# raulmur/ORB_SLAM2

Hardware: NVIDIA H100
Metric: stereo frames/sec (ORB extract L+R + ComputeStereoMatches, KITTI-shaped 1242x375 @2000 kpts) (higher is better)
Workload: dtype u8

## Files before the change

orb_slam2_b200/csrc/k_fast.cu:

```cuda
#include <cuda.h>

#include <cstring>

#include "borb_internal.h"

#include <algorithm>
#include <vector>

namespace borb {

namespace {

constexpr int TP = 160;
constexpr int TROWS = 66;
constexpr int QCAP = 60 * 128;

__device__ __forceinline__ uint32_t smem_u32(const void* p) { return (uint32_t)__cvta_generic_to_shared(p); }

template <int DX>
__device__ __forceinline__ uint32_t win(uint32_t W0, uint32_t W1, uint32_t W2) {
    if (DX == 0) return W1;
    if (DX > 0) return __byte_perm(W1, W2, DX | ((DX + 1) << 4) | ((DX + 2) << 8) | ((DX + 3) << 12));
    constexpr int K = 4 + DX;
    return __byte_perm(W0, W1, K | ((K + 1) << 4) | ((K + 2) << 8) | ((K + 3) << 12));
}

__device__ __forceinline__ uint32_t gt_flag(uint32_t q, uint32_t v, uint32_t K) {
    const uint32_t a = __vabsdiffu4(q, v);
    return (a + K) | a;
}

__device__ __forceinline__ uint32_t score_word(const uint32_t (&R0)[7], const uint32_t (&R1)[7], const uint32_t (&R2)[7]) {
#define ROWJ(dy) R0[(dy) + 3], R1[(dy) + 3], R2[(dy) + 3]
    uint32_t wn[16];
    wn[0] = win<0>(ROWJ(3));    wn[1] = win<1>(ROWJ(3));    wn[2] = win<2>(ROWJ(2));     wn[3] = win<3>(ROWJ(1));
    wn[4] = win<3>(ROWJ(0));    wn[5] = win<3>(ROWJ(-1));   wn[6] = win<2>(ROWJ(-2));    wn[7] = win<1>(ROWJ(-3));
    wn[8] = win<0>(ROWJ(-3));   wn[9] = win<-1>(ROWJ(-3));  wn[10] = win<-2>(ROWJ(-2));  wn[11] = win<-3>(ROWJ(-1));
    wn[12] = win<-3>(ROWJ(0));  wn[13] = win<-3>(ROWJ(1));  wn[14] = win<-2>(ROWJ(2));   wn[15] = win<-1>(ROWJ(3));
#undef ROWJ
    const uint32_t v = R1[3];
    uint32_t res[2];
#pragma unroll
    for (int half = 0; half < 2; half++) {
        const uint32_t v2 = half ? __byte_perm(v, 0u, 0x4341) : (v & 0x00FF00FFu);
        const uint32_t nv2 = __vneg2(v2);
        uint32_t d[16];
#pragma unroll
        for (int k = 0; k < 16; k++) {
            const uint32_t q2 = half ? __byte_perm(wn[k], 0u, 0x4341) : (wn[k] & 0x00FF00FFu);
            d[k] = __vadd2(q2, nv2);
        }
        uint32_t lo3[16], hi3[16];
#pragma unroll
        for (int k = 0; k < 16; k++) {
            lo3[k] = __vimin3_s16x2(d[k], d[(k + 1) & 15], d[(k + 2) & 15]);
            hi3[k] = __vimax3_s16x2(d[k], d[(k + 1) & 15], d[(k + 2) & 15]);
        }
        uint32_t lo9[16], hi9[16];
#pragma unroll
        for (int k = 0; k < 16; k++) {
            lo9[k] = __vimin3_s16x2(lo3[k], lo3[(k + 3) & 15], lo3[(k + 6) & 15]);
            hi9[k] = __vimax3_s16x2(hi3[k], hi3[(k + 3) & 15], hi3[(k + 6) & 15]);
        }
        uint32_t bb[5], dd[5];
#pragma unroll
        for (int k = 0; k < 5; k++) {
            bb[k] = __vimax3_s16x2(lo9[3 * k], lo9[3 * k + 1], lo9[3 * k + 2]);
            dd[k] = __vimin3_s16x2(hi9[3 * k], hi9[3 * k + 1], hi9[3 * k + 2]);
        }
        const uint32_t bright = __vimax3_s16x2(__vimax3_s16x2(bb[0], bb[1], bb[2]), __vimax3_s16x2(bb[3], bb[4], lo9[15]), bb[0]);
        const uint32_t darkm = __vimin3_s16x2(__vimin3_s16x2(dd[0], dd[1], dd[2]), __vimin3_s16x2(dd[3], dd[4], hi9[15]), dd[0]);
        res[half] = __viaddmax_s16x2_relu(__vmaxs2(bright, __vneg2(darkm)), 0xFFFFFFFFu, 0u);
    }
    return res[1] * 256u + res[0];
}

}

struct TMaps { CUtensorMap m[BORB_MAX_LEVELS]; };

struct __align__(16) FastTile { int16_t l, ncell, x0, x1, y0, y1, wCell, hCell; };

__global__ void __launch_bounds__(256, 4) fast_kernel(const __grid_constant__ Geometry g, const __grid_constant__ TMaps tm,
                                                   const FastTile* __restrict__ tiles, uint32_t* __restrict__ cand, int* __restrict__ cand_cnt) {
    __shared__ __align__(128) uint8_t tile[TROWS * TP];
    __shared__ __align__(16) uint8_t score[60 * TP];
    __shared__ uint16_t queue[QCAP];
    __shared__ uint16_t wqueue[8 * 256];
    __shared__ int wcnt[8];
    __shared__ __align__(8) unsigned long long bar;
    __shared__ uint32_t scoredRow[60];
    __shared__ int qn, needB;
    __shared__ int cellHasIni[128 / 30 + 1];
    __shared__ uint8_t cellOf[128];

    const int img = blockIdx.y;
    const FastTile T = tiles[blockIdx.x];
    const int l = T.l, ncell = T.ncell, x0 = T.x0, x1 = T.x1, y0 = T.y0, y1 = T.y1;
    const int wCell = T.wCell, hCell = T.hCell;
    const LevelGeom& L = g.lv[l];
    const int tw = x1 - x0, th = y1 - y0;
    const int tid = threadIdx.x;
    const int lane = tid & 31, wrp = tid >> 5;

    const int xs = (x0 - 4) & ~15;
    const int off = x0 - xs;
    if (tid == 0) {
        asm volatile("mbarrier.init.shared::cta.b64 [%0], 1;" ::"r"(smem_u32(&bar)));
        asm volatile("fence.mbarrier_init.release.cluster;" ::: "memory");
        const uint32_t bytes = (uint32_t)TP * (uint32_t)(hCell + 6);
        asm volatile("mbarrier.arrive.expect_tx.shared::cta.b64 _, [%0], %1;" ::"r"(smem_u32(&bar)), "r"(bytes) : "memory");
        asm volatile(
            "cp.async.bulk.tensor.3d.shared::cluster.global.tile.mbarrier::complete_tx::bytes [%0], [%1, {%2, %3, %4}], [%5];"
            ::"r"(smem_u32(tile)), "l"(reinterpret_cast<uint64_t>(&tm.m[l])), "r"(xs), "r"(y0 - 3), "r"(img), "r"(smem_u32(&bar))
            : "memory");
    }
    if (tid < 128 / 30 + 1) cellHasIni[tid] = 0;
    if (tid < 128) cellOf[tid] = (uint8_t)(tid / wCell);
    if (tid == 0) { qn = 0; needB = 0; }
    __syncthreads();
    asm volatile(
        "{\n"
        ".reg .pred p;\n"
        "FAST_TMA_WAIT:\n"
        "mbarrier.try_wait.parity.shared::cta.b64 p, [%0], 0;\n"
        "@p bra FAST_TMA_DONE;\n"
        "bra FAST_TMA_WAIT;\n"
        "FAST_TMA_DONE:\n"
        "}\n" ::"r"(smem_u32(&bar))
        : "memory");
    if (g.fast_mode == 1) {
        if (reinterpret_cast<const uint32_t*>(tile)[tid] == 0x12345678u && cand_cnt[0] == -1) cand[0] = 1;
        return;
    }

    const int tlow = g.ini_th;
    const uint32_t* T32 = reinterpret_cast<const uint32_t*>(tile);
    uint32_t* S32 = reinterpret_cast<uint32_t*>(score);
    const int wbase = off >> 2;
    const uint32_t T1 = (uint32_t)(127 - min(tlow, 127)) * 0x01010101u;
    const uint32_t TC = (uint32_t)min(max(tlow, 1), 128) * 0x01010101u;
    const bool reject_ok = tlow <= 127;

    auto commit = [&](uint32_t sw, int yy, int wc, bool write, int tlow, uint32_t TC, uint32_t needMask) {
        const int col = 4 * wc;
        uint32_t vm = 0;
#pragma unroll
        for (int b = 0; b < 4; b++)
            if (col + b - off >= 0 && col + b - off < tw) vm |= 0x80u << (8 * b);
        if (write) S32[yy * (TP / 4) + wc] = sw;
        uint32_t m = (((sw | 0x80808080u) - TC) | sw) & vm & needMask;
        if (tlow > 128) {
            m = 0;
#pragma unroll
            for (int b = 0; b < 4; b++)
                if ((int)((sw >> (8 * b)) & 0xFF) >= tlow) m |= 0x80u << (8 * b);
            m &= vm & needMask;
        }
        if (!write) m = 0;
        const unsigned any = __ballot_sync(0xFFFFFFFFu, m != 0);
        if (any) {
            const int c = __popc(m);
            int incl = c;
#pragma unroll
            for (int o2 = 1; o2 < 32; o2 <<= 1) {
                const int t = __shfl_up_sync(0xFFFFFFFFu, incl, o2);
                if (lane >= o2) incl += t;
            }
            int base = 0;
            if (lane == 31) base = atomicAdd(&qn, incl);
            base = __shfl_sync(0xFFFFFFFFu, base, 31) + incl - c;
            uint32_t mm = m;
            while (mm) {
                const int b = (__ffs(mm) - 1) >> 3;
                mm &= mm - 1;
                queue[base++] = (uint16_t)((yy << 8) | (col + b));
            }
        }
    };

    {
        const int RG = (th + 7) >> 3;
        const int yBeg = wrp * RG, yEnd = min(th, yBeg + RG);
        const int wc = wbase + lane;
        uint32_t vmask = 0;
#pragma unroll
        for (int b = 0; b < 4; b++)
            if (4 * wc + b - off >= 0 && 4 * wc + b - off < tw) vmask |= 0x80u << (8 * b);
        uint32_t a0[7], a1[7], a2[7];
        int wcount = 0;
        if (yBeg < yEnd) {
#pragma unroll
            for (int j = 0; j < 6; j++) {
                const uint32_t* rp = T32 + (yBeg + j) * (TP / 4) + wc - 1;
                a0[j] = rp[0]; a1[j] = rp[1]; a2[j] = rp[2];
            }
        }
#pragma unroll
        for (int it = 0; it < 8; it++) {
            const int yy = yBeg + it;
            if (yy < yEnd) {
                {
                    const uint32_t* rp = T32 + (yy + 6) * (TP / 4) + wc - 1;
                    a0[(it + 6) % 7] = rp[0]; a1[(it + 6) % 7] = rp[1]; a2[(it + 6) % 7] = rp[2];
                }
#define ROW(dy) a0[(it + (dy) + 3) % 7], a1[(it + (dy) + 3) % 7], a2[(it + (dy) + 3) % 7]
                bool keep = vmask != 0;
                if (reject_ok && keep) {
                    const uint32_t v = a1[(it + 3) % 7];
                    uint32_t acc = gt_flag(win<0>(ROW(3)), v, T1) | gt_flag(win<0>(ROW(-3)), v, T1);
                    acc &= gt_flag(win<2>(ROW(2)), v, T1) | gt_flag(win<-2>(ROW(-2)), v, T1);
                    acc &= gt_flag(win<3>(ROW(0)), v, T1) | gt_flag(win<-3>(ROW(0)), v, T1);
                    acc &= gt_flag(win<2>(ROW(-2)), v, T1) | gt_flag(win<-2>(ROW(2)), v, T1);
                    keep = (acc & vmask) != 0;
                }
#undef ROW
                const unsigned bal = __ballot_sync(0xFFFFFFFFu, keep);
                if (lane == 0) scoredRow[yy] = bal;
                if (!keep && vmask != 0) S32[yy * (TP / 4) + wc] = 0;
                if (keep) wqueue[wrp * 256 + wcount + __popc(bal & ((1u << lane) - 1))] = (uint16_t)((yy << 5) | lane);
                wcount += __popc(bal);
            }
        }
        if (lane == 0) wcnt[wrp] = wcount;
    }
    __syncthreads();
    if (g.fast_mode == 2) {
        if (wcnt[0] == -1) cand[0] = 1;
        return;
    }

    {
        int c[8], nw = 0;
#pragma unroll
        for (int w = 0; w < 8; w++) { c[w] = wcnt[w]; nw += c[w]; }
        for (int eb = 0; eb < nw; eb += 256) {
            const int e = eb + tid;
            uint32_t sw = 0;
            int yy = 0, wc = wbase;
            const bool have = e < nw;
            if (have) {
                int seg = 0, r = e;
#pragma unroll
                for (int w = 0; w < 7; w++)
                    if (seg == w && r >= c[w]) { r -= c[w]; seg = w + 1; }
                const int we = wqueue[seg * 256 + r];
                yy = we >> 5;
                wc = wbase + (we & 31);
                uint32_t R0[7], R1[7], R2[7];
#pragma unroll
                for (int j = 0; j < 7; j++) {
                    const uint32_t* rp = T32 + (yy + j) * (TP / 4) + wc - 1;
                    R0[j] = rp[0]; R1[j] = rp[1]; R2[j] = rp[2];
                }
                sw = score_word(R0, R1, R2);
            }
            commit(sw, yy, wc, have, tlow, TC, 0xFFFFFFFFu);
        }
    }
    __syncthreads();
    int nq = qn;
    if (g.fast_mode == 3) {
        if (nq == -1) cand[0] = 1;
        return;
    }

    uint32_t* out = cand + (size_t)img * g.cand_image_stride + L.cand_off;
    int* cnt = cand_cnt + img * g.nlevels + l;

    auto nms = [&](int n, bool mark) {
        for (int e = tid; e < n; e += 256) {
            const int q = queue[e];
            const int col = q & 255, yy = q >> 8;
            const int xx = col - off;
            const int s = score[yy * TP + col];
            const int c = cellOf[xx];
            const int cx0 = c * wCell, cx1 = min(cx0 + wCell, tw);
            bool ismax = true;
#pragma unroll
            for (int dy = -1; dy <= 1; dy++)
#pragma unroll
                for (int dx = -1; dx <= 1; dx++) {
                    if (dx == 0 && dy == 0) continue;
                    const int qx = xx + dx, qy = yy + dy;
                    if (qx < cx0 || qx >= cx1 || qy < 0 || qy >= th) continue;
                    if (!(s > (int)score[qy * TP + col + dx])) ismax = false;
                }
            if (ismax) {
                if (mark) cellHasIni[c] = 1;
            } else
                queue[e] = 0xFFFF;
        }
    };
    auto emit = [&](int n) {
        for (int eb = 0; eb < n; eb += 256) {
            const int e = eb + tid;
            int s = 0, xx = 0, yy = 0;
            if (e < n) {
                const int q = queue[e];
                if (q != 0xFFFF) {
                    const int col = q & 255;
                    yy = q >> 8; xx = col - off;
                    s = score[yy * TP + col];
                }
            }
            const unsigned m = __ballot_sync(0xFFFFFFFFu, s > 0);
            if (m) {
                int base = 0;
                if (lane == 0) base = atomicAdd(cnt, __popc(m));
                base = __shfl_sync(0xFFFFFFFFu, base, 0);
                if (s > 0) {
                    const int pos = base + __popc(m & ((1u << lane) - 1));
                    if (pos < L.cand_cap) out[pos] = pack_xys(x0 + xx, y0 + yy, s);
                }
            }
        }
    };

    nms(nq, true);
    __syncthreads();
    emit(nq);
    if (tid < ncell && tid * wCell < tw && !cellHasIni[tid] && g.min_th < g.ini_th) needB = 1;
    __syncthreads();
    if (!needB) return;

    {
        if (tid == 0) qn = 0;
        __syncthreads();
        const int tmin = g.min_th;
        const uint32_t T1b = (uint32_t)(127 - min(tmin, 127)) * 0x01010101u;
        const uint32_t TCb = (uint32_t)min(max(tmin, 1), 128) * 0x01010101u;
        const int nwords = th * 32;
        for (int wb = 0; wb < nwords; wb += 256) {
            const int widx = wb + tid;
            const int yy = widx >> 5;
            const int wc = wbase + (widx & 31);
            uint32_t needMask = 0, sw = 0;
            bool write = false;
            if (widx < nwords) {
#pragma unroll
                for (int b = 0; b < 4; b++) {
                    const int xx = 4 * wc + b - off;
                    if (xx >= 0 && xx < tw && !cellHasIni[cellOf[xx]]) needMask |= 0x80u << (8 * b);
                }
                if (needMask) {
                    write = true;
                    if ((scoredRow[yy] >> (widx & 31)) & 1u) {
                        sw = S32[yy * (TP / 4) + wc];
                    } else {
                        uint32_t R0[7], R1[7], R2[7];
#pragma unroll
                        for (int j = 0; j < 7; j++) {
                            const uint32_t* rp = T32 + (yy + j) * (TP / 4) + wc - 1;
                            R0[j] = rp[0]; R1[j] = rp[1]; R2[j] = rp[2];
                        }
                        bool keep = true;
                        if (tmin <= 127) {
                            const uint32_t v = R1[3];
#define ROWJ(dy) R0[(dy) + 3], R1[(dy) + 3], R2[(dy) + 3]
                            uint32_t acc = gt_flag(win<0>(ROWJ(3)), v, T1b) | gt_flag(win<0>(ROWJ(-3)), v, T1b);
                            acc &= gt_flag(win<2>(ROWJ(2)), v, T1b) | gt_flag(win<-2>(ROWJ(-2)), v, T1b);
                            acc &= gt_flag(win<3>(ROWJ(0)), v, T1b) | gt_flag(win<-3>(ROWJ(0)), v, T1b);
                            acc &= gt_flag(win<2>(ROWJ(-2)), v, T1b) | gt_flag(win<-2>(ROWJ(2)), v, T1b);
#undef ROWJ
                            keep = (acc & 0x80808080u) != 0;
                        }
                        sw = keep ? score_word(R0, R1, R2) : 0u;
                    }
                }
            }
            commit(sw, yy, wc, write, tmin, TCb, needMask);
        }
        __syncthreads();
        nq = qn;
        nms(nq, false);
        __syncthreads();
        emit(nq);
    }
}

typedef CUresult (*EncodeTiledFn)(CUtensorMap*, CUtensorMapDataType, cuuint32_t, void*, const cuuint64_t*, const cuuint64_t*,
                                  const cuuint32_t*, const cuuint32_t*, CUtensorMapInterleave, CUtensorMapSwizzle,
                                  CUtensorMapL2promotion, CUtensorMapFloatOOBfill);

borb_status build_fast_tmaps(const Geometry& g, const Workspace& ws, void* out_tmaps) {
    static EncodeTiledFn encode = nullptr;
    if (!encode) {
        void* fn = nullptr;
        cudaDriverEntryPointQueryResult qres;
        cudaError_t e = cudaGetDriverEntryPoint("cuTensorMapEncodeTiled", &fn, cudaEnableDefault, &qres);
        if (e != cudaSuccess || qres != cudaDriverEntryPointSuccess || !fn) {
            set_error("cuTensorMapEncodeTiled unavailable (%s)", cudaGetErrorString(e));
            return BORB_ERR_CUDA;
        }
        encode = (EncodeTiledFn)fn;
    }
    TMaps* tm = reinterpret_cast<TMaps*>(out_tmaps);
    std::memset(tm, 0, sizeof(TMaps));
    for (int l = 0; l < g.nlevels; l++) {
        const LevelGeom& L = g.lv[l];
        cuuint64_t dims[3] = {(cuuint64_t)L.w, (cuuint64_t)L.h, (cuuint64_t)ws.max_images};
        cuuint64_t strides[2] = {(cuuint64_t)L.pitch, (cuuint64_t)g.pyr_image_stride};
        cuuint32_t box[3] = {(cuuint32_t)TP, (cuuint32_t)(L.hCell + 6), 1};
        cuuint32_t estr[3] = {1, 1, 1};
        CUresult r = encode(&tm->m[l], CU_TENSOR_MAP_DATA_TYPE_UINT8, 3, ws.pyr + L.pyr_off, dims, strides, box, estr,
                            CU_TENSOR_MAP_INTERLEAVE_NONE, CU_TENSOR_MAP_SWIZZLE_NONE, CU_TENSOR_MAP_L2_PROMOTION_L2_128B,
                            CU_TENSOR_MAP_FLOAT_OOB_FILL_NONE);
        if (r != CUDA_SUCCESS) {
            set_error("cuTensorMapEncodeTiled failed for level %d (CUresult %d)", l, (int)r);
            return BORB_ERR_CUDA;
        }
    }
    return BORB_OK;
}

size_t fast_tmaps_bytes() { return sizeof(TMaps); }

borb_status build_fast_tiles(const Geometry& g, Workspace& ws) {
    std::vector<FastTile> t;
    for (int l = 0; l < g.nlevels; l++) {
        const LevelGeom& L = g.lv[l];
        for (int cellRow = 0; cellRow < L.nRows; cellRow++)
            for (int blkCol = 0; blkCol < L.blkCols; blkCol++) {
                const int cell0 = blkCol * L.cellsPerBlk;
                const int ncell = std::min(L.cellsPerBlk, L.nCols - cell0);
                const int x0 = EDGE + cell0 * L.wCell, x1 = std::min(x0 + ncell * L.wCell, L.w - EDGE);
                const int y0 = EDGE + cellRow * L.hCell, y1 = std::min(y0 + L.hCell, L.h - EDGE);
                if (x0 >= x1 || y0 >= y1) continue;
                FastTile f;
                f.l = (int16_t)l; f.ncell = (int16_t)ncell; f.x0 = (int16_t)x0; f.x1 = (int16_t)x1; f.y0 = (int16_t)y0; f.y1 = (int16_t)y1;
                f.wCell = (int16_t)L.wCell; f.hCell = (int16_t)L.hCell;
                t.push_back(f);
            }
    }
    cudaFree(ws.fast_tiles); ws.fast_tiles = nullptr;
    ws.fast_n_tiles = (int)t.size();
    if (t.empty()) return BORB_OK;
    BORB_CUDA(cudaMalloc(&ws.fast_tiles, t.size() * sizeof(FastTile)));
    BORB_CUDA(cudaMemcpy(ws.fast_tiles, t.data(), t.size() * sizeof(FastTile), cudaMemcpyHostToDevice));
    return BORB_OK;
}

int launch_fast(const Geometry& g, const Workspace& ws, int n_images, cudaStream_t s) {
    if (ws.fast_n_tiles == 0) return 0;
    dim3 grid(ws.fast_n_tiles, n_images);
    fast_kernel<<<grid, 256, 0, s>>>(g, *reinterpret_cast<const TMaps*>(ws.fast_tmaps), reinterpret_cast<const FastTile*>(ws.fast_tiles), ws.cand, ws.cand_cnt);
    return 1;
}

}
```

Before: 35610.

## Score FAST corners per surviving pixel instead of per 4-pixel word

FAST scoring is restructured. The old path scored whole 4-byte words whenever any pixel in the word passed the rejection test. The new path records per-pixel survivor flags in a warp queue, compacts the individual pixels into a block-wide queue, and scores two pixels per thread with a scalar 16-bit pair routine reading bytes from shared memory. The low-threshold pass reuses the same collect/score path and drops the scoredRow cache, so previously scored words are recomputed. This cuts wasted scoring on non-candidate pixels but adds an extra compaction stage, byte-granular shared loads and extra block syncs inside the scoring loop.

```diff
diff --git a/orb_slam2_b200/csrc/k_fast.cu b/orb_slam2_b200/csrc/k_fast.cu
--- a/orb_slam2_b200/csrc/k_fast.cu
+++ b/orb_slam2_b200/csrc/k_fast.cu
@@ -30,49 +30,40 @@
     return (a + K) | a;
 }
 
-__device__ __forceinline__ uint32_t score_word(const uint32_t (&R0)[7], const uint32_t (&R1)[7], const uint32_t (&R2)[7]) {
-#define ROWJ(dy) R0[(dy) + 3], R1[(dy) + 3], R2[(dy) + 3]
-    uint32_t wn[16];
-    wn[0] = win<0>(ROWJ(3));    wn[1] = win<1>(ROWJ(3));    wn[2] = win<2>(ROWJ(2));     wn[3] = win<3>(ROWJ(1));
-    wn[4] = win<3>(ROWJ(0));    wn[5] = win<3>(ROWJ(-1));   wn[6] = win<2>(ROWJ(-2));    wn[7] = win<1>(ROWJ(-3));
-    wn[8] = win<0>(ROWJ(-3));   wn[9] = win<-1>(ROWJ(-3));  wn[10] = win<-2>(ROWJ(-2));  wn[11] = win<-3>(ROWJ(-1));
-    wn[12] = win<-3>(ROWJ(0));  wn[13] = win<-3>(ROWJ(1));  wn[14] = win<-2>(ROWJ(2));   wn[15] = win<-1>(ROWJ(3));
-#undef ROWJ
-    const uint32_t v = R1[3];
-    uint32_t res[2];
-#pragma unroll
-    for (int half = 0; half < 2; half++) {
-        const uint32_t v2 = half ? __byte_perm(v, 0u, 0x4341) : (v & 0x00FF00FFu);
-        const uint32_t nv2 = __vneg2(v2);
-        uint32_t d[16];
-#pragma unroll
-        for (int k = 0; k < 16; k++) {
-            const uint32_t q2 = half ? __byte_perm(wn[k], 0u, 0x4341) : (wn[k] & 0x00FF00FFu);
-            d[k] = __vadd2(q2, nv2);
-        }
-        uint32_t lo3[16], hi3[16];
-#pragma unroll
-        for (int k = 0; k < 16; k++) {
-            lo3[k] = __vimin3_s16x2(d[k], d[(k + 1) & 15], d[(k + 2) & 15]);
-            hi3[k] = __vimax3_s16x2(d[k], d[(k + 1) & 15], d[(k + 2) & 15]);
-        }
-        uint32_t lo9[16], hi9[16];
-#pragma unroll
-        for (int k = 0; k < 16; k++) {
-            lo9[k] = __vimin3_s16x2(lo3[k], lo3[(k + 3) & 15], lo3[(k + 6) & 15]);
-            hi9[k] = __vimax3_s16x2(hi3[k], hi3[(k + 3) & 15], hi3[(k + 6) & 15]);
-        }
-        uint32_t bb[5], dd[5];
-#pragma unroll
-        for (int k = 0; k < 5; k++) {
-            bb[k] = __vimax3_s16x2(lo9[3 * k], lo9[3 * k + 1], lo9[3 * k + 2]);
-            dd[k] = __vimin3_s16x2(hi9[3 * k], hi9[3 * k + 1], hi9[3 * k + 2]);
-        }
-        const uint32_t bright = __vimax3_s16x2(__vimax3_s16x2(bb[0], bb[1], bb[2]), __vimax3_s16x2(bb[3], bb[4], lo9[15]), bb[0]);
-        const uint32_t darkm = __vimin3_s16x2(__vimin3_s16x2(dd[0], dd[1], dd[2]), __vimin3_s16x2(dd[3], dd[4], hi9[15]), dd[0]);
-        res[half] = __viaddmax_s16x2_relu(__vmaxs2(bright, __vneg2(darkm)), 0xFFFFFFFFu, 0u);
-    }
-    return res[1] * 256u + res[0];
+__device__ __forceinline__ uint32_t score_pair(const uint32_t (&d)[16], uint32_t v2) {
+    uint32_t lo3[16], hi3[16];
+#pragma unroll
+    for (int k = 0; k < 16; k++) {
+        lo3[k] = __vimin3_s16x2(d[k], d[(k + 1) & 15], d[(k + 2) & 15]);
+        hi3[k] = __vimax3_s16x2(d[k], d[(k + 1) & 15], d[(k + 2) & 15]);
+    }
+    uint32_t lo9[16], hi9[16];
+#pragma unroll
+    for (int k = 0; k < 16; k++) {
+        lo9[k] = __vimin3_s16x2(lo3[k], lo3[(k + 3) & 15], lo3[(k + 6) & 15]);
+        hi9[k] = __vimax3_s16x2(hi3[k], hi3[(k + 3) & 15], hi3[(k + 6) & 15]);
+    }
+    uint32_t bb[5], dd[5];
+#pragma unroll
+    for (int k = 0; k < 5; k++) {
+        bb[k] = __vimax3_s16x2(lo9[3 * k], lo9[3 * k + 1], lo9[3 * k + 2]);
+        dd[k] = __vimin3_s16x2(hi9[3 * k], hi9[3 * k + 1], hi9[3 * k + 2]);
+    }
+    const uint32_t bright = __vimax3_s16x2(__vimax3_s16x2(bb[0], bb[1], bb[2]), __vimax3_s16x2(bb[3], bb[4], lo9[15]), bb[0]);
+    const uint32_t darkm = __vimin3_s16x2(__vimin3_s16x2(dd[0], dd[1], dd[2]), __vimin3_s16x2(dd[3], dd[4], hi9[15]), dd[0]);
+    return __viaddmax_s16x2_relu(__vmaxs2(__vsub2(bright, v2), __vsub2(v2, darkm)), 0xFFFFFFFFu, 0u);
+}
+
+__device__ __forceinline__ uint32_t score_pixels(const uint8_t* pa, const uint8_t* pb) {
+    constexpr int RX[16] = {0, 1, 2, 3, 3, 3, 2, 1, 0, -1, -2, -3, -3, -3, -2, -1};
+    constexpr int RY[16] = {3, 3, 2, 1, 0, -1, -2, -3, -3, -3, -2, -1, 0, 1, 2, 3};
+    uint32_t d[16];
+#pragma unroll
+    for (int k = 0; k < 16; k++) {
+        const int o = RY[k] * TP + RX[k];
+        d[k] = (uint32_t)pa[o] | ((uint32_t)pb[o] << 16);
+    }
+    return score_pair(d, (uint32_t)pa[0] | ((uint32_t)pb[0] << 16));
 }
 
 }
@@ -86,11 +77,9 @@
     __shared__ __align__(128) uint8_t tile[TROWS * TP];
     __shared__ __align__(16) uint8_t score[60 * TP];
     __shared__ uint16_t queue[QCAP];
-    __shared__ uint16_t wqueue[8 * 256];
-    __shared__ int wcnt[8];
+    __shared__ uint32_t wqueue[8 * 256];
     __shared__ __align__(8) unsigned long long bar;
-    __shared__ uint32_t scoredRow[60];
-    __shared__ int qn, needB;
+    __shared__ int pn, qn, needB;
     __shared__ int cellHasIni[128 / 30 + 1];
     __shared__ uint8_t cellOf[128];
 
@@ -117,7 +106,7 @@
     }
     if (tid < 128 / 30 + 1) cellHasIni[tid] = 0;
     if (tid < 128) cellOf[tid] = (uint8_t)(tid / wCell);
-    if (tid == 0) { qn = 0; needB = 0; }
+    if (tid == 0) { pn = 0; qn = 0; needB = 0; }
     __syncthreads();
     asm volatile(
         "{\n"
@@ -134,59 +123,21 @@
         return;
     }
 
-    const int tlow = g.ini_th;
     const uint32_t* T32 = reinterpret_cast<const uint32_t*>(tile);
     uint32_t* S32 = reinterpret_cast<uint32_t*>(score);
     const int wbase = off >> 2;
-    const uint32_t T1 = (uint32_t)(127 - min(tlow, 127)) * 0x01010101u;
-    const uint32_t TC = (uint32_t)min(max(tlow, 1), 128) * 0x01010101u;
-    const bool reject_ok = tlow <= 127;
-
-    auto commit = [&](uint32_t sw, int yy, int wc, bool write, int tlow, uint32_t TC, uint32_t needMask) {
-        const int col = 4 * wc;
-        uint32_t vm = 0;
-#pragma unroll
-        for (int b = 0; b < 4; b++)
-            if (col + b - off >= 0 && col + b - off < tw) vm |= 0x80u << (8 * b);
-        if (write) S32[yy * (TP / 4) + wc] = sw;
-        uint32_t m = (((sw | 0x80808080u) - TC) | sw) & vm & needMask;
-        if (tlow > 128) {
-            m = 0;
-#pragma unroll
-            for (int b = 0; b < 4; b++)
-                if ((int)((sw >> (8 * b)) & 0xFF) >= tlow) m |= 0x80u << (8 * b);
-            m &= vm & needMask;
-        }
-        if (!write) m = 0;
-        const unsigned any = __ballot_sync(0xFFFFFFFFu, m != 0);
-        if (any) {
-            const int c = __popc(m);
-            int incl = c;
-#pragma unroll
-            for (int o2 = 1; o2 < 32; o2 <<= 1) {
-                const int t = __shfl_up_sync(0xFFFFFFFFu, incl, o2);
-                if (lane >= o2) incl += t;
-            }
-            int base = 0;
-            if (lane == 31) base = atomicAdd(&qn, incl);
-            base = __shfl_sync(0xFFFFFFFFu, base, 31) + incl - c;
-            uint32_t mm = m;
-            while (mm) {
-                const int b = (__ffs(mm) - 1) >> 3;
-                mm &= mm - 1;
-                queue[base++] = (uint16_t)((yy << 8) | (col + b));
-            }
-        }
-    };
-
-    {
+    const int wc = wbase + lane;
+    uint32_t vmask = 0;
+#pragma unroll
+    for (int b = 0; b < 4; b++)
+        if (4 * wc + b - off >= 0 && 4 * wc + b - off < tw) vmask |= 0x80u << (8 * b);
+
+    auto collect = [&](int t, uint32_t m, bool zero) {
+        const uint32_t K = (uint32_t)(127 - min(t, 127)) * 0x01010101u;
+        asm volatile("" : "+r"(m));
+        const bool reject = t <= 127;
         const int RG = (th + 7) >> 3;
         const int yBeg = wrp * RG, yEnd = min(th, yBeg + RG);
-        const int wc = wbase + lane;
-        uint32_t vmask = 0;
-#pragma unroll
-        for (int b = 0; b < 4; b++)
-            if (4 * wc + b - off >= 0 && 4 * wc + b - off < tw) vmask |= 0x80u << (8 * b);
         uint32_t a0[7], a1[7], a2[7];
         int wcount = 0;
         if (yBeg < yEnd) {
@@ -205,59 +156,84 @@
                     a0[(it + 6) % 7] = rp[0]; a1[(it + 6) % 7] = rp[1]; a2[(it + 6) % 7] = rp[2];
                 }
 #define ROW(dy) a0[(it + (dy) + 3) % 7], a1[(it + (dy) + 3) % 7], a2[(it + (dy) + 3) % 7]
-                bool keep = vmask != 0;
-                if (reject_ok && keep) {
+                uint32_t f = m;
+                if (reject && m) {
                     const uint32_t v = a1[(it + 3) % 7];
-                    uint32_t acc = gt_flag(win<0>(ROW(3)), v, T1) | gt_flag(win<0>(ROW(-3)), v, T1);
-                    acc &= gt_flag(win<2>(ROW(2)), v, T1) | gt_flag(win<-2>(ROW(-2)), v, T1);
-                    acc &= gt_flag(win<3>(ROW(0)), v, T1) | gt_flag(win<-3>(ROW(0)), v, T1);
-                    acc &= gt_flag(win<2>(ROW(-2)), v, T1) | gt_flag(win<-2>(ROW(2)), v, T1);
-                    keep = (acc & vmask) != 0;
+                    uint32_t acc = gt_flag(win<0>(ROW(3)), v, K) | gt_flag(win<0>(ROW(-3)), v, K);
+                    acc &= gt_flag(win<2>(ROW(2)), v, K) | gt_flag(win<-2>(ROW(-2)), v, K);
+                    acc &= gt_flag(win<3>(ROW(0)), v, K) | gt_flag(win<-3>(ROW(0)), v, K);
+                    acc &= gt_flag(win<2>(ROW(-2)), v, K) | gt_flag(win<-2>(ROW(2)), v, K);
+                    f = acc & m;
                 }
 #undef ROW
-                const unsigned bal = __ballot_sync(0xFFFFFFFFu, keep);
-                if (lane == 0) scoredRow[yy] = bal;
-                if (!keep && vmask != 0) S32[yy * (TP / 4) + wc] = 0;
-                if (keep) wqueue[wrp * 256 + wcount + __popc(bal & ((1u << lane) - 1))] = (uint16_t)((yy << 5) | lane);
+                const unsigned bal = __ballot_sync(0xFFFFFFFFu, f != 0);
+                if (zero && m != 0) S32[yy * (TP / 4) + wc] = 0;
+                if (f) wqueue[wrp * 256 + wcount + __popc(bal & ((1u << lane) - 1))] = f | (uint32_t)(yy << 8) | (uint32_t)wc;
                 wcount += __popc(bal);
             }
         }
-        if (lane == 0) wcnt[wrp] = wcount;
-    }
+        __syncwarp();
+        for (int i = 0; i < wcount; i += 32) {
+            const uint32_t we = i + lane < wcount ? wqueue[wrp * 256 + i + lane] : 0u;
+            const uint32_t fl = we & 0x80808080u;
+            const int c = __popc(fl);
+            int incl = c;
+#pragma unroll
+            for (int o2 = 1; o2 < 32; o2 <<= 1) {
+                const int s = __shfl_up_sync(0xFFFFFFFFu, incl, o2);
+                if (lane >= o2) incl += s;
+            }
+            int base = 0;
+            if (lane == 31) base = atomicAdd(&pn, incl);
+            base = __shfl_sync(0xFFFFFFFFu, base, 31) + incl - c;
+            const int e = (int)((we >> 8) & 63) << 8 | (int)(4 * (we & 127));
+#pragma unroll
+            for (int b = 0; b < 4; b++)
+                if (fl & (0x80u << (8 * b))) queue[base++] = (uint16_t)(e + b);
+        }
+    };
+
+    auto score_queue = [&](int t) {
+        const int np = pn;
+        const int tc = max(t, 1);
+        for (int rb = 0; rb < np; rb += 512) {
+            const int e0 = rb + wrp * 64 + lane, e1 = e0 + 32;
+            const bool va = e0 < np, vb = e1 < np;
+            const int qa = va ? queue[e0] : off;
+            const int qb = vb ? queue[e1] : qa;
+            __syncthreads();
+            if (rb + wrp * 64 < np) {
+                const int ia = (qa >> 8) * TP + (qa & 255), ib = (qb >> 8) * TP + (qb & 255);
+                const uint32_t s2 = score_pixels(tile + ia + 3 * TP, tile + ib + 3 * TP);
+                const int sa = (int)(s2 & 0xFFFFu), sb = (int)(s2 >> 16);
+                if (va) score[ia] = (uint8_t)sa;
+                if (vb) score[ib] = (uint8_t)sb;
+                const bool ca = va && sa >= tc, cb = vb && sb >= tc;
+                if (__any_sync(0xFFFFFFFFu, ca || cb)) {
+                    const int c = (int)ca + (int)cb;
+                    int incl = c;
+#pragma unroll
+                    for (int o2 = 1; o2 < 32; o2 <<= 1) {
+                        const int s = __shfl_up_sync(0xFFFFFFFFu, incl, o2);
+                        if (lane >= o2) incl += s;
+                    }
+                    int base = 0;
+                    if (lane == 31) base = atomicAdd(&qn, incl);
+                    base = __shfl_sync(0xFFFFFFFFu, base, 31) + incl - c;
+                    if (ca) queue[base++] = (uint16_t)qa;
+                    if (cb) queue[base] = (uint16_t)qb;
+                }
+            }
+        }
+    };
+
+    collect(g.ini_th, vmask, true);
     __syncthreads();
     if (g.fast_mode == 2) {
-        if (wcnt[0] == -1) cand[0] = 1;
+        if (pn == -1) cand[0] = 1;
         return;
     }
-
-    {
-        int c[8], nw = 0;
-#pragma unroll
-        for (int w = 0; w < 8; w++) { c[w] = wcnt[w]; nw += c[w]; }
-        for (int eb = 0; eb < nw; eb += 256) {
-            const int e = eb + tid;
-            uint32_t sw = 0;
-            int yy = 0, wc = wbase;
-            const bool have = e < nw;
-            if (have) {
-                int seg = 0, r = e;
-#pragma unroll
-                for (int w = 0; w < 7; w++)
-                    if (seg == w && r >= c[w]) { r -= c[w]; seg = w + 1; }
-                const int we = wqueue[seg * 256 + r];
-                yy = we >> 5;
-                wc = wbase + (we & 31);
-                uint32_t R0[7], R1[7], R2[7];
-#pragma unroll
-                for (int j = 0; j < 7; j++) {
-                    const uint32_t* rp = T32 + (yy + j) * (TP / 4) + wc - 1;
-                    R0[j] = rp[0]; R1[j] = rp[1]; R2[j] = rp[2];
-                }
-                sw = score_word(R0, R1, R2);
-            }
-            commit(sw, yy, wc, have, tlow, TC, 0xFFFFFFFFu);
-        }
-    }
+    score_queue(g.ini_th);
     __syncthreads();
     int nq = qn;
     if (g.fast_mode == 3) {
@@ -325,52 +301,17 @@
     if (!needB) return;
 
     {
-        if (tid == 0) qn = 0;
+        uint32_t need = 0;
+#pragma unroll
+        for (int b = 0; b < 4; b++) {
+            const int xx = 4 * wc + b - off;
+            if (xx >= 0 && xx < tw && !cellHasIni[cellOf[xx]]) need |= 0x80u << (8 * b);
+        }
+        if (tid == 0) { pn = 0; qn = 0; }
         __syncthreads();
-        const int tmin = g.min_th;
-        const uint32_t T1b = (uint32_t)(127 - min(tmin, 127)) * 0x01010101u;
-        const uint32_t TCb = (uint32_t)min(max(tmin, 1), 128) * 0x01010101u;
-        const int nwords = th * 32;
-        for (int wb = 0; wb < nwords; wb += 256) {
-            const int widx = wb + tid;
-            const int yy = widx >> 5;
-            const int wc = wbase + (widx & 31);
-            uint32_t needMask = 0, sw = 0;
-            bool write = false;
-            if (widx < nwords) {
-#pragma unroll
-                for (int b = 0; b < 4; b++) {
-                    const int xx = 4 * wc + b - off;
-                    if (xx >= 0 && xx < tw && !cellHasIni[cellOf[xx]]) needMask |= 0x80u << (8 * b);
-                }
-                if (needMask) {
-                    write = true;
-                    if ((scoredRow[yy] >> (widx & 31)) & 1u) {
-                        sw = S32[yy * (TP / 4) + wc];
-                    } else {
-                        uint32_t R0[7], R1[7], R2[7];
-#pragma unroll
-                        for (int j = 0; j < 7; j++) {
-                            const uint32_t* rp = T32 + (yy + j) * (TP / 4) + wc - 1;
-                            R0[j] = rp[0]; R1[j] = rp[1]; R2[j] = rp[2];
-                        }
-                        bool keep = true;
-                        if (tmin <= 127) {
-                            const uint32_t v = R1[3];
-#define ROWJ(dy) R0[(dy) + 3], R1[(dy) + 3], R2[(dy) + 3]
-                            uint32_t acc = gt_flag(win<0>(ROWJ(3)), v, T1b) | gt_flag(win<0>(ROWJ(-3)), v, T1b);
-                            acc &= gt_flag(win<2>(ROWJ(2)), v, T1b) | gt_flag(win<-2>(ROWJ(-2)), v, T1b);
-                            acc &= gt_flag(win<3>(ROWJ(0)), v, T1b) | gt_flag(win<-3>(ROWJ(0)), v, T1b);
-                            acc &= gt_flag(win<2>(ROWJ(-2)), v, T1b) | gt_flag(win<-2>(ROWJ(2)), v, T1b);
-#undef ROWJ
-                            keep = (acc & 0x80808080u) != 0;
-                        }
-                        sw = keep ? score_word(R0, R1, R2) : 0u;
-                    }
-                }
-            }
-            commit(sw, yy, wc, write, tmin, TCb, needMask);
-        }
+        collect(g.min_th, need, false);
+        __syncthreads();
+        score_queue(g.min_th);
         __syncthreads();
         nq = qn;
         nms(nq, false);
```

Measured after the change: 37570 (median of 6 runs). 5.5% higher.
